# dusk-network/plonk_gadgets

Measured on AMD Instinct MI355X. Metric: gadget constraints/sec (range_check 256-bit), higher is better.
Workload: dtype u64x4 (BLS12-381 scalar, Montgomery limbs)

## Files before the change

plonk_gadgets_amd/csrc/emit.hpp:

```cpp
#pragma once

#include <type_traits>

#include "fr.hpp"

namespace pg {

constexpr int kThreads = 256;

union FrVec {
    Fr f;
    uint4 v[2];
};

struct EmitOut {
    uint4 *q[5];
    uint64_t *w[3];
    uint4 *vars;
    uint64_t gate_base, var_base;
    uint64_t zero_var;
    const uint64_t *row_off;
    const uint64_t *var_off;
    uint64_t batch;
    uint32_t tiles;
    uint32_t stride_rows;
    const uint4 *inv_dense;
    uint64_t inv_elems;
    uint32_t inv_in_place;
    uint32_t early_span, early_tiles;
};
__device__ __forceinline__ bool early_rows_candidate(const EmitOut &O, uint64_t w0, uint32_t Wt, uint32_t W, uint64_t &s0, uint64_t &s1) {
    s0 = s1 = 0;
    if (!O.early_tiles || Wt != W) return false;
    s0 = w0 - w0 % O.early_span;
    s1 = s0 + O.early_span < O.batch ? s0 + O.early_span : O.batch;
    return (w0 - s0) / W < O.early_tiles;
}

__device__ __forceinline__ void fetch_inverse(const EmitOut &O, uint64_t s, void *rec_fr) {
    uint4 *z = reinterpret_cast<uint4 *>(rec_fr);
    z[0] = O.inv_dense[s];
    z[1] = O.inv_dense[O.inv_elems + s];
}

enum : uint32_t { T_ZERO = 0, T_ONE = 1, T_NEG1 = 2, T_QC_A = 3, T_QC_B = 4, T_POW = 8 };
constexpr int kTableEntries = 8 + 256;

typedef unsigned int pg_u32x4 __attribute__((ext_vector_type(4)));

__device__ __forceinline__ void store16(uint4 *p, uint4 v) {
#if defined(PG_NT_STORES)
    pg_u32x4 t = {v.x, v.y, v.z, v.w};
    __builtin_nontemporal_store(t, reinterpret_cast<pg_u32x4 *>(p));
#else
    *p = v;
#endif
}

__device__ __forceinline__ void lds_barrier() {
#if defined(PG_FULL_BARRIERS)
    __syncthreads();
#else
    asm volatile("s_waitcnt lgkmcnt(0)\n\ts_barrier" ::: "memory");
#endif
}

__device__ __forceinline__ uint64_t uniform64(uint64_t x) {
    return (uint64_t)(uint32_t)__builtin_amdgcn_readfirstlane((int)(uint32_t)x) |
           (uint64_t)(uint32_t)__builtin_amdgcn_readfirstlane((int)(uint32_t)(x >> 32)) << 32;
}

__device__ __forceinline__ Fr lds_fr(const uint4 *table, uint32_t id) {
    FrVec t;
    t.v[0] = table[2 * id];
    t.v[1] = table[2 * id + 1];
    return t.f;
}

__device__ __forceinline__ void fill_common_table(uint4 *table, const uint4 *pow2, uint32_t tid, uint32_t entries) {
    for (uint32_t e = tid; e < entries; e += kThreads) {
        FrVec t;
        t.f = fr_zero();
        if (e == T_ONE) t.f = fr_one();
        else if (e == T_NEG1) t.f = fr_neg_one();
        else if (e >= T_POW && pow2) { t.v[0] = pow2[(e - T_POW) * 2]; t.v[1] = pow2[(e - T_POW) * 2 + 1]; }
        if (e != T_QC_A && e != T_QC_B) {
            table[2 * e] = t.v[0];
            table[2 * e + 1] = t.v[1];
        }
    }
}

template <bool SMALL_ITEMS, uint32_t UNI>
__device__ __forceinline__ uint32_t find_item(const uint32_t *off, uint32_t Wt, uint32_t r, uint32_t it, bool uniform) {
    if constexpr (UNI != 0) {
        if (uniform) return r / UNI;
    }
    if constexpr (SMALL_ITEMS) {
        uint32_t lo = it, hi = Wt;
        while (hi - lo > 1) {
            const uint32_t mid = (lo + hi) >> 1;
            if (off[mid] <= r) lo = mid; else hi = mid;
        }
        return lo;
    } else {
        while (r >= off[it + 1]) it++;
        return it;
    }
}

template <class GD, bool RAGGED = GD::kRagged>
struct UniformShape {
    static constexpr uint32_t rows = 0, vars = 0;
};
template <class GD>
struct UniformShape<GD, true> {
    static constexpr uint32_t rows = GD::kUniformRows, vars = GD::kUniformVars;
};

template <class GD, class = void>
struct Periodic {
    static constexpr bool ok = false;
};
template <class GD>
struct Periodic<GD, std::void_t<decltype(GD::kPeriodic)>> {
    static constexpr bool ok = GD::kPeriodic;
};
constexpr uint32_t periodic_wire_lanes(uint32_t R) {
    uint32_t L = 256;
    while ((2 * L) % R) L--;
    return L;
}

#ifndef PG_EMIT_WAVES_PER_SIMD
#define PG_EMIT_WAVES_PER_SIMD 1
#endif

enum EmitMode : int { EMIT_ALL = 0, EMIT_STRUCTURE = 1, EMIT_ROWS = 2, EMIT_VALUES = 3 };

template <class GD, class = void>
struct Split {
    static constexpr bool ok = false;
};
template <class GD>
struct Split<GD, std::void_t<decltype(GD::kSplit)>> {
    static constexpr bool ok = GD::kSplit;
};
template <class GD, class = void>
struct RegionVars {
    static constexpr bool ok = false;
};
template <class GD>
struct RegionVars<GD, std::void_t<decltype(GD::kRegionVars)>> {
    static constexpr bool ok = GD::kRegionVars;
};
template <class GD, class = void>
struct InvDense {
    static constexpr bool ok = false;
};
template <class GD>
struct InvDense<GD, std::void_t<decltype(GD::kInvDense)>> {
    static constexpr bool ok = GD::kInvDense;
};
template <class GD, int MODE>
struct EmitShape {
    using Rec = typename GD::ItemRec;
    static constexpr int W = GD::W;
};
template <class GD>
struct EmitShape<GD, EMIT_ROWS> {
    using Rec = typename GD::RowRec;
    static constexpr int W = GD::kRowsW;
};

constexpr uint32_t kRegionLead = 8, kRegionStage = (kRegionLead + 256 + 16) / 8 * 9;

template <class GD, int MODE = EMIT_ALL>
__global__ __launch_bounds__(kThreads, PG_EMIT_WAVES_PER_SIMD) void emit_kernel(const typename GD::Args A, const EmitOut O) {
    static_assert(MODE != EMIT_STRUCTURE || !(GD::kRagged || GD::kRecInRows), "rows of this gadget depend on its inputs");
    constexpr bool kVars = MODE == EMIT_ALL || MODE == EMIT_VALUES;
    constexpr bool kRows = MODE != EMIT_VALUES;
    constexpr int W = EmitShape<GD, MODE>::W;
    using Rec = typename EmitShape<GD, MODE>::Rec;
    constexpr uint32_t kTable = GD::kUsePow2 ? kTableEntries : T_POW;
    __shared__ uint4 s_table[kTable * 2];
    __shared__ Rec s_item[W];
    __shared__ uint32_t s_roff[W + 1], s_voff[W + 1];

    const uint32_t tid = threadIdx.x;
    {
        const uint4 *p2 = nullptr;
        if constexpr (GD::kUsePow2) p2 = GD::pow2(A);
        fill_common_table(s_table, p2, tid, kTable);
    }
    GD::fill_table(A, s_table, tid);
    lds_barrier();

    for (uint32_t t = blockIdx.x; t < O.tiles; t += gridDim.x) {
#if defined(PG_XCD_REMAP)
        const uint32_t q8 = O.tiles >> 3, r8 = O.tiles & 7, x = t & 7, k = t >> 3;
        const uint32_t tile = x * q8 + (x < r8 ? x : r8) + k;
#elif defined(PG_TILE_SPREAD)
        const uint32_t qs = O.tiles / PG_TILE_SPREAD, rs = O.tiles % PG_TILE_SPREAD, x = t % PG_TILE_SPREAD, k = t / PG_TILE_SPREAD;
        const uint32_t tile = x * qs + (x < rs ? x : rs) + k;
#else
        const uint32_t tile = t;
#endif
        const uint64_t w0 = O.stride_rows ? (uint64_t)tile : (uint64_t)tile * W;
        const uint32_t Wt = O.stride_rows ? 1u : (uint32_t)((O.batch - w0) < (uint64_t)W ? (O.batch - w0) : (uint64_t)W);
        if constexpr (MODE == EMIT_ROWS && Periodic<GD>::ok) {
            if (O.row_off[w0 + Wt] - O.row_off[w0] == (uint64_t)Wt * UniformShape<GD>::rows) continue;
        }
        uint64_t row0, var0;
        uint32_t G = 0, V = 0;
        uint64_t my_r = 0, my_v = 0, tail_r = 0, tail_v = 0;
        if constexpr (GD::kRagged) {
            row0 = O.row_off[w0];
            var0 = O.var_off[w0];
            if (tid <= Wt) {
                my_r = O.row_off[w0 + tid];
                my_v = O.var_off[w0 + tid];
            }
            if constexpr (W == kThreads) {
                if (tid == 0) {
                    tail_r = O.row_off[w0 + Wt];
                    tail_v = O.var_off[w0 + Wt];
                }
            }
        } else {
            G = GD::rows_per_item(A);
            V = GD::vars_per_item(A);
            row0 = w0 * (O.stride_rows ? O.stride_rows : G);
            var0 = w0 * V;
        }

        if constexpr ((GD::kRagged || GD::kRecInRows) && MODE != EMIT_STRUCTURE) {
            for (uint32_t i = tid; i < Wt; i += kThreads) GD::item_rows(A, O, w0 + i, s_table, s_item[i]);
        }
        if constexpr (GD::kRagged) {
            if (tid <= Wt) {
                s_roff[tid] = (uint32_t)(my_r - row0);
                s_voff[tid] = (uint32_t)(my_v - var0);
            }
            if constexpr (W == kThreads) {
                if (tid == 0) {
                    s_roff[Wt] = (uint32_t)(tail_r - row0);
                    s_voff[Wt] = (uint32_t)(tail_v - var0);
                }
            }
        }
        if constexpr (GD::kRagged || GD::kRecInRows) lds_barrier();
        if constexpr (kVars) {
            if (tid < Wt) GD::item(A, O, w0 + tid, s_table, s_item[tid]);
        }

        const uint32_t total_rows = GD::kRagged ? s_roff[Wt] : Wt * G;
        const uint32_t total_vars = GD::kRagged ? s_voff[Wt] : Wt * V;
        constexpr uint32_t kUniR = UniformShape<GD>::rows, kUniV = UniformShape<GD>::vars;
        const bool uni_rows = kUniR != 0 && total_rows == Wt * kUniR, uni_vars = kUniV != 0 && total_vars == Wt * kUniV;

        if constexpr (kRows) {
            {
                const uint32_t total = total_rows * 2;
#if defined(PG_UNALIGNED_SWEEPS)
                const uint32_t mis = 0;
#else
                const uint32_t mis = (uint32_t)((reinterpret_cast<uintptr_t>(O.q[0] + row0 * 2) >> 4) & 7u);
#endif
                const uint32_t v0 = tid < mis ? tid + kThreads : tid;
                const uint32_t h = (v0 - mis) & 1;
                uint32_t it = 0, j = (v0 - mis) >> 1;
                if constexpr (!GD::kRagged) { it = j / G; j -= it * G; }
                for (uint32_t u = v0; u < total + mis; u += kThreads) {
                    const uint32_t idx = u - mis;
                    if constexpr (GD::kRagged) {
                        const uint32_t r = idx >> 1;
                        it = find_item<W >= 64, kUniR>(s_roff, Wt, r, it, uni_rows);
                        j = uni_rows ? r - it * kUniR : r - s_roff[it];
                    }
                    uint4 v[5];
                    GD::selectors(A, s_item[it], j, s_table, h, v);
#pragma unroll
                    for (int c = 0; c < 5; c++) store16(O.q[c] + (row0 * 2 + idx), v[c]);
                    if constexpr (!GD::kRagged) {
                        j += kThreads / 2;
                        if (j >= G) { const uint32_t d = j / G; it += d; j -= d * G; }
                    }
                }
            }

#pragma unroll
            for (int c = 0; c < 3; c++) {
                uint64_t *col = O.w[c] + row0;
                const uint32_t shift = (uint32_t)((reinterpret_cast<uintptr_t>(col) >> 3) & 1);
                const uint32_t pairs = (total_rows + shift + 1) >> 1;
#if defined(PG_UNALIGNED_SWEEPS)
                const uint32_t pmis = 0;
#else
                const uint32_t pmis = (uint32_t)(((reinterpret_cast<uintptr_t>(col) - 8 * shift) >> 4) & 7u);
#endif
                uint32_t it = 0;
                for (uint32_t pv = tid < pmis ? tid + kThreads : tid; pv < pairs + pmis; pv += kThreads) {
                    const uint32_t p = pv - pmis;
                    const int64_t r0 = (int64_t)2 * p - shift;
                    uint64_t val[2];
#pragma unroll
                    for (int k = 0; k < 2; k++) {
                        const int64_t r = r0 + k;
                        uint32_t rr = r < 0 ? 0u : (uint32_t)r;
                        if (rr >= total_rows) rr = total_rows - 1;
                        uint32_t j, vo;
                        if constexpr (GD::kRagged) {
                            it = find_item<W >= 64, kUniR>(s_roff, Wt, rr, it, uni_rows);
                            j = uni_rows ? rr - it * kUniR : rr - s_roff[it];
                            vo = (uni_rows && uni_vars) ? it * kUniV : s_voff[it];
                        } else {
                            it = rr / G;
                            j = rr - it * G;
                            vo = it * V;
                        }
                        uint64_t out[3];
                        GD::wires(A, O, s_item[it], w0 + it, O.var_base + var0 + vo, j, out);
                        val[k] = out[c];
                    }
                    if (r0 >= 0 && r0 + 1 < (int64_t)total_rows) {
                        store16(reinterpret_cast<uint4 *>(col + r0),
                                make_uint4((uint32_t)val[0], (uint32_t)(val[0] >> 32), (uint32_t)val[1],
                                           (uint32_t)(val[1] >> 32)));
                    } else {
                        if (r0 >= 0) col[r0] = val[0];
                        if (r0 + 1 < (int64_t)total_rows) col[r0 + 1] = val[1];
                    }
                }
            }
        }

        lds_barrier();

        if constexpr (kVars) {
            const bool inv_here = InvDense<GD>::ok && !O.inv_in_place;
#if defined(PG_UNALIGNED_SWEEPS)
            const uint32_t smis = 0;
#else
            const uint32_t smis = (uint32_t)((reinterpret_cast<uintptr_t>(O.vars + var0 * 2) >> 5) & 3u);
#endif
#if !defined(PG_VAR_SWEEP_SINGLE)
            if constexpr (RegionVars<GD>::ok && MODE == EMIT_VALUES) {
                __shared__ uint4 s_reg[4 * kRegionStage];
                const uint32_t wave = tid >> 6, lane = tid & 63;
                uint4 *wp = s_reg + wave * kRegionStage;
                constexpr uint32_t B2 = 2 * GD::kBlocks;
                const uint32_t units = Wt * B2;
                const uint32_t tile_mis = (uint32_t)((reinterpret_cast<uintptr_t>(O.vars + var0 * 2) >> 5) & 3u);
                for (uint32_t q = wave; q < units; q += kThreads / 64) {
                    const uint32_t it = q / B2, r = q - it * B2, b = r >> 1;
                    const uint32_t kind = (r + (GD::kBlocks == 2 ? it : it >> 1)) & 1;
                    const Rec &R = s_item[it];
                    const auto &Bk = GD::region_block(R, b);
                    const uint32_t n = GD::region_n(A, R);
                    const uint32_t count = kind ? (n + 1 < 256 ? n + 1 : 256) : 256;
                    uint32_t vitem, vend;
                    if constexpr (GD::kRagged) {
                        vitem = uni_vars ? it * kUniV : s_voff[it];
                        vend = uni_vars ? vitem + kUniV : s_voff[it + 1];
                    } else {
                        vitem = it * V;
                        vend = vitem + V;
                    }
                    const uint32_t kfirst = GD::region_k(A, R, b, kind ? 257 : 1);
                    const uint32_t mis0 = (tile_mis + vitem) & 3u;
                    uint32_t ks, ke;
                    if (kind == 0) {
                        ks = b == 0 ? 0 : kfirst;
                        if (it != 0 || b != 0) ks += (4u - ((mis0 + ks) & 3u)) & 3u;
                        ke = kfirst + 256;
                        ke -= (mis0 + ke) & 3u;
                    } else {
                        ks = kfirst - ((mis0 + kfirst) & 3u);
                        ke = b + 1 < GD::kBlocks ? GD::region_k(A, R, b + 1, 1) : vend - vitem;
                        if (it + 1 != Wt || b + 1 < GD::kBlocks) ke += (4u - ((mis0 + ke) & 3u)) & 3u;
                    }
                    const uint32_t h_end = (count - 1) >> 7;
                    uint32_t hole = ~0u;
                    if (!inv_here)
                        for (uint32_t k = kfirst + count; k < ke && k < vend - vitem; k++)
                            if (GD::is_inv_slot(A, R, k)) hole = k;
                    FrVec v[4];
                    const uint32_t i0 = 4 * lane;
                    if (kind == 0) {
#pragma unroll
                        for (int t = 0; t < 4; t++) v[t].f = raw_bit(Bk.Tc, i0 + t) ? fr_one() : fr_zero();
                    } else {
                        v[0].f = fr_zero();
                        if (i0 && i0 < count) v[0].f = fr_to_mont(raw_low_bits(Bk.Tc, i0));
#pragma unroll
                        for (int t = 1; t < 4; t++) {
                            v[t].f = v[t - 1].f;
                            if (i0 + t < count && raw_bit(Bk.Tc, i0 + t - 1)) {
                                FrVec p;
                                p.v[0] = s_table[2 * (T_POW + i0 + t - 1)];
                                p.v[1] = s_table[2 * (T_POW + i0 + t - 1) + 1];
                                v[t].f = fr_add(v[t - 1].f, p.f);
                            }
                        }
                    }
                    const uint32_t npre = ks < kfirst ? kfirst - ks : 0, npost = ke > kfirst + count ? ke - (kfirst + count) : 0;
                    FrVec nb;
                    uint32_t nb_at = ~0u;
                    if (lane < npre + npost) {
                        const uint32_t k = lane < npre ? ks + lane : kfirst + count + (lane - npre);
                        const uint32_t vitem_n = vend - vitem;
                        nb.f = k < vitem_n ? GD::var_value(A, R, s_table, k) : GD::var_value(A, s_item[it + 1], s_table, k - vitem_n);
                        nb_at = kRegionLead + 2 * (k - kfirst) - (lane < npre ? 0 : 256 * h_end);
                    }
#pragma unroll
                    for (int h = 0; h < 2; h++) {
                        if ((lane >> 5) == (uint32_t)h) {
                            const uint32_t u0 = kRegionLead + 8 * (lane & 31), w0 = u0 + (u0 >> 3);
#pragma unroll
                            for (int t = 0; t < 4; t++) {
                                wp[w0 + 2 * t] = v[t].v[0];
                                wp[w0 + 2 * t + 1] = v[t].v[1];
                            }
                        }
                        if (h == 1 && lane == 31) {
#pragma unroll
                            for (int t = 0; t < 4; t++) {
                                wp[kRegionLead - 8 + 2 * t] = v[t].v[0];
                                wp[kRegionLead - 8 + 2 * t + 1] = v[t].v[1];
                            }
                        }
                        if (nb_at != ~0u && (lane < npre ? h == 0 : (uint32_t)h == h_end)) {
                            wp[nb_at + (nb_at >> 3)] = nb.v[0];
                            wp[nb_at + 1 + ((nb_at + 1) >> 3)] = nb.v[1];
                        }
                        asm volatile("" ::: "memory");
                        const uint32_t mid = kfirst + 128 - ((mis0 + kfirst + 128) & 3u);
                        const uint32_t lo = h == 0 ? ks : mid, hi = (uint32_t)h == h_end ? ke : (h == 0 ? mid : lo);
                        const uint32_t total = hi > lo ? 2 * (hi - lo) : 0;
                        uint4 *dst = O.vars + ((uint64_t)var0 + vitem + lo) * 2;
                        const uint32_t mis = (uint32_t)((reinterpret_cast<uintptr_t>(dst) >> 4) & 7u);
                        const uint32_t lead = kRegionLead + 2 * (lo - kfirst) - 256 * h;
#pragma unroll
                        for (int j = 0; j < 5; j++) {
                            const uint32_t g = 64 * j + lane - mis;
                            const uint32_t u = g + lead;
                            if (g < total && lo + (g >> 1) != hole) store16(dst + g, wp[u + (u >> 3)]);
                        }
                        asm volatile("" ::: "memory");
                    }
                }
            } else
#endif
            {
            const uint32_t sv0 = tid < smis ? tid + kThreads : tid;
                uint32_t it = 0, k = sv0 - smis;
                if constexpr (!GD::kRagged) { it = k / V; k -= it * V; }
                for (uint32_t sv = sv0; sv < total_vars + smis; sv += kThreads) {
                    const uint32_t s = sv - smis;
                    if constexpr (GD::kRagged) {
                        it = find_item<W >= 64, kUniV>(s_voff, Wt, s, it, uni_vars);
                        k = uni_vars ? s - it * kUniV : s - s_voff[it];
                    }
                    uint4 *dst = O.vars + (var0 + s) * 2;
                    if (inv_here || !GD::is_inv_slot(A, s_item[it], k)) {
                        FrVec val;
                        val.f = GD::var_value(A, s_item[it], s_table, k);
                        store16(dst, val.v[0]);
                        store16(dst + 1, val.v[1]);
                    }
                    if constexpr (!GD::kRagged) {
                        k += kThreads;
                        if (k >= V) { const uint32_t d = k / V; it += d; k -= d * V; }
                    }
                }
            }
            }
        lds_barrier();
    }
}

#ifndef PG_ROWS_WAVES_PER_SIMD
#define PG_ROWS_WAVES_PER_SIMD 8
#endif
template <class GD>
__device__ __forceinline__ void periodic_tile_rows(const typename GD::Args &A, const EmitOut &O, const uint4 v[5], uint32_t tid, uint64_t w0,
                                                   uint32_t Wt, uint64_t row0, uint64_t var0) {
    constexpr uint32_t R = GD::kUniformRows, VV = GD::kUniformVars;
    constexpr uint32_t IPP = (kThreads / 2) / R, LS = IPP * R * 2;
    constexpr uint32_t LW = periodic_wire_lanes(R), IPW = 2 * LW / R;
    typename GD::RowRec full{};
    const uint32_t total_rows = Wt * R;
    if (tid < LS) {
        const uint32_t passes = (total_rows * 2 + LS - 1) / LS;
        uint4 *base[5];
        uint32_t at[5];
#pragma unroll
        for (int c = 0; c < 5; c++) {
            base[c] = O.q[c] + (row0 * 2 + tid);
            at[c] = (uint32_t)(((uint64_t)c * passes) / 5);
        }
        for (uint32_t p = 0; p < passes; p++) {
#pragma unroll
            for (int c = 0; c < 5; c++) {
                const uint32_t off = at[c] * LS;
                if (off + tid < total_rows * 2) store16(base[c] + off, v[c]);
                at[c] = at[c] + 1 == passes ? 0 : at[c] + 1;
            }
        }
    }
#pragma unroll
    for (int c = 0; c < 3; c++) {
        uint64_t *col = O.w[c] + row0;
        const uint32_t shift = (uint32_t)((reinterpret_cast<uintptr_t>(col) >> 3) & 1);
        if (tid < LW) {
            uint64_t wbase[2], slope[2];
#pragma unroll
            for (int k = 0; k < 2; k++) {
                const int32_t r = (int32_t)(2 * tid + k) - (int32_t)shift;
                const int32_t it = r < 0 ? -1 : r / (int32_t)R;
                const uint32_t j = (uint32_t)(r - it * (int32_t)R);
                const uint64_t vb = O.var_base + var0 + (uint64_t)(int64_t)it * VV;
                uint64_t a[3], b[3];
                GD::wires(A, O, full, w0 + (uint64_t)(int64_t)it, vb, j, a);
                GD::wires(A, O, full, w0 + (uint64_t)(int64_t)it, vb + 1, j, b);
                wbase[k] = a[c];
                slope[k] = b[c] - a[c];
            }
            const uint64_t step = (uint64_t)IPW * VV;
            uint64_t adv = 0;
            for (int64_t r0 = (int64_t)2 * tid - shift; r0 < (int64_t)total_rows; r0 += 2 * LW, adv += step) {
                const uint64_t v0 = wbase[0] + slope[0] * adv, v1 = wbase[1] + slope[1] * adv;
                if (r0 >= 0 && r0 + 1 < (int64_t)total_rows) {
                    store16(reinterpret_cast<uint4 *>(col + r0),
                            make_uint4((uint32_t)v0, (uint32_t)(v0 >> 32), (uint32_t)v1, (uint32_t)(v1 >> 32)));
                } else {
                    if (r0 >= 0) col[r0] = v0;
                    if (r0 + 1 < (int64_t)total_rows) col[r0 + 1] = v1;
                }
            }
        }
    }
}
template <class GD>
__device__ __forceinline__ void periodic_lane_selectors(const typename GD::Args &A, const uint4 *table, uint32_t tid, uint4 v[5]) {
    constexpr uint32_t R = GD::kUniformRows, IPP = (kThreads / 2) / R, LS = IPP * R * 2;
    typename GD::RowRec full{};
    const uint32_t rl = (tid < LS ? tid : 0) >> 1;
    GD::selectors(A, full, rl - (rl / R) * R, table, tid & 1, v);
}

template <class GD>
__global__ __launch_bounds__(kThreads, PG_ROWS_WAVES_PER_SIMD) void rows_periodic_kernel(const typename GD::Args A, const EmitOut O) {
    constexpr int W = GD::kRowsW;
    constexpr uint32_t R = GD::kUniformRows;
    __shared__ uint4 s_table[T_POW * 2];
    const uint32_t tid = threadIdx.x;
#if defined(PG_ROWS_SETPRIO)
    __builtin_amdgcn_s_setprio(PG_ROWS_SETPRIO);
#endif
    fill_common_table(s_table, nullptr, tid, T_POW);
    GD::fill_table(A, s_table, tid);
    lds_barrier();
    uint4 v[5];
    periodic_lane_selectors<GD>(A, s_table, tid, v);

    for (uint32_t tile = blockIdx.x; tile < O.tiles; tile += gridDim.x) {
        const uint64_t w0 = (uint64_t)tile * W;
        const uint32_t Wt = (uint32_t)((O.batch - w0) < (uint64_t)W ? (O.batch - w0) : (uint64_t)W);
        uint64_t s0, s1;
        const bool cand = early_rows_candidate(O, w0, Wt, W, s0, s1);
        const uint64_t span_rows = cand ? O.row_off[s1] - O.row_off[s0] : 0;
        const uint64_t row0 = uniform64(O.row_off[w0]), var0 = uniform64(O.var_off[w0]), row1 = uniform64(O.row_off[w0 + Wt]);
        if (row1 - row0 != Wt * R) continue;
        if (cand && uniform64(span_rows) == (s1 - s0) * R) continue;
        periodic_tile_rows<GD>(A, O, v, tid, w0, Wt, row0, var0);
    }
}

__global__ __launch_bounds__(kThreads) void fill_kernel(uint4 *dst, uint64_t n16, uint32_t streams, uint64_t pattern) {
    const uint4 v = make_uint4((uint32_t)pattern, (uint32_t)(pattern >> 32), (uint32_t)~pattern, (uint32_t)(~pattern >> 32));
    const uint64_t part = n16 / streams;
    constexpr uint64_t kPiece = 65536;
    for (uint64_t base = (uint64_t)blockIdx.x * kPiece; base < part; base += (uint64_t)gridDim.x * kPiece) {
        const uint64_t end = base + kPiece < part ? base + kPiece : part;
        for (uint64_t i = base + threadIdx.x; i < end; i += kThreads)
            for (uint32_t s = 0; s < streams; s++) store16(dst + (uint64_t)s * part + i, v);
    }
    if (blockIdx.x == 0)
        for (uint64_t i = part * streams + threadIdx.x; i < n16; i += kThreads) store16(dst + i, v);
}

constexpr uint32_t kFillOneshotLds = 160 * 1024 / 2 - 1024;
constexpr uint32_t kFillOneshotUnits = 2 * kThreads;
__global__ __launch_bounds__(kThreads) void fill_oneshot_kernel(uint4 *dst, uint64_t n16, uint64_t pattern) {
    extern __shared__ uint4 fill_oneshot_pad[];
    const uint4 v = make_uint4((uint32_t)pattern, (uint32_t)(pattern >> 32), (uint32_t)~pattern, (uint32_t)(~pattern >> 32));
    const uint64_t base = (uint64_t)blockIdx.x * kFillOneshotUnits + threadIdx.x;
#pragma unroll
    for (uint32_t k = 0; k < kFillOneshotUnits / kThreads; k++)
        if (base + k * kThreads < n16) store16(dst + base + k * kThreads, v);
    if (n16 == ~0ull) fill_oneshot_pad[threadIdx.x] = v;
}

__global__ __launch_bounds__(kThreads) void fill_columns_kernel(EmitOut O, uint64_t n_gates, uint64_t n_vars, uint64_t rows_per_tile,
                                                                uint64_t vars_per_tile, uint64_t pattern) {
    const uint4 v = make_uint4((uint32_t)pattern, (uint32_t)(pattern >> 32), (uint32_t)~pattern, (uint32_t)(~pattern >> 32));
    for (uint64_t tile = blockIdx.x; tile < O.tiles; tile += gridDim.x) {
        const uint64_t r0 = tile * rows_per_tile, r1 = r0 + rows_per_tile < n_gates ? r0 + rows_per_tile : n_gates;
        const uint64_t v0 = tile * vars_per_tile, v1 = tile + 1 == O.tiles ? n_vars : (v0 + vars_per_tile < n_vars ? v0 + vars_per_tile : n_vars);
        if (r0 < r1) {
            for (uint64_t u = 2 * r0 + threadIdx.x; u < 2 * r1; u += kThreads) {
#pragma unroll
                for (int c = 0; c < 5; c++) store16(O.q[c] + u, v);
            }
            for (uint64_t u = r0 / 2 + threadIdx.x; u < r1 / 2; u += kThreads) {
#pragma unroll
                for (int c = 0; c < 3; c++) store16(reinterpret_cast<uint4 *>(O.w[c]) + u, v);
            }
            if ((r1 & 1) && threadIdx.x == 0)
                for (int c = 0; c < 3; c++) O.w[c][r1 - 1] = pattern;
        }
        for (uint64_t u = 2 * v0 + threadIdx.x; u < 2 * v1; u += kThreads) store16(O.vars + u, v);
    }
}

__global__ __launch_bounds__(kThreads) void from_canonical_kernel(const uint4 *raw, uint64_t n, uint4 *out, uint8_t *bad_mask,
                                                                 uint32_t *bad_count) {
    const uint64_t i = (uint64_t)blockIdx.x * kThreads + threadIdx.x;
    if (i >= n) return;
    FrVec x;
    x.v[0] = raw[2 * i];
    x.v[1] = raw[2 * i + 1];
    const Fr q = fr_modulus();
    bool ge = true;
    for (int k = 3; k >= 0; k--)
        if (x.f.l[k] != q.l[k]) { ge = x.f.l[k] > q.l[k]; break; }
    FrVec r;
    r.f = ge ? fr_zero() : fr_to_mont(x.f);
    out[2 * i] = r.v[0];
    out[2 * i + 1] = r.v[1];
    if (bad_mask) bad_mask[i] = ge ? 1 : 0;
    if (ge) atomicAdd(bad_count, 1u);
}
__global__ __launch_bounds__(kThreads) void to_canonical_kernel(const uint4 *in, uint64_t n, uint4 *raw) {
    const uint64_t i = (uint64_t)blockIdx.x * kThreads + threadIdx.x;
    if (i >= n) return;
    FrVec x, r;
    x.v[0] = in[2 * i];
    x.v[1] = in[2 * i + 1];
    r.f = fr_from_mont(x.f);
    raw[2 * i] = r.v[0];
    raw[2 * i + 1] = r.v[1];
}

constexpr int kScanBlock = 1024;

__device__ __forceinline__ uint64_t block_exclusive_scan(uint64_t v, uint64_t *s_warp, uint64_t &block_total) {
    const uint32_t lane = threadIdx.x & 63, wave = threadIdx.x >> 6;
    uint64_t incl = v;
#pragma unroll
    for (int d = 1; d < 64; d <<= 1) {
        uint64_t t = __shfl_up(incl, d, 64);
        if (lane >= (uint32_t)d) incl += t;
    }
    if (lane == 63) s_warp[wave] = incl;
    __syncthreads();
    uint64_t base = 0;
    for (uint32_t wv = 0; wv < wave; wv++) base += s_warp[wv];
    block_total = s_warp[0] + s_warp[1] + s_warp[2] + s_warp[3];
    __syncthreads();
    return base + incl - v;
}

__global__ __launch_bounds__(kThreads) void scan_top_kernel(uint64_t *blk_rows, uint64_t *blk_vars, uint32_t nblk) {
    __shared__ uint64_t s_warp[4];
    uint64_t carry_r = 0, carry_v = 0;
    for (uint32_t base = 0; base < nblk; base += kThreads) {
        uint32_t i = base + threadIdx.x;
        uint64_t r = i < nblk ? blk_rows[i] : 0, v = i < nblk ? blk_vars[i] : 0, tr, tv;
        uint64_t er = block_exclusive_scan(r, s_warp, tr);
        uint64_t ev = block_exclusive_scan(v, s_warp, tv);
        if (i < nblk) { blk_rows[i] = carry_r + er; blk_vars[i] = carry_v + ev; }
        carry_r += tr;
        carry_v += tv;
    }
}

struct PlanTotals {
    uint64_t n_gates, n_vars;
    uint32_t errs, pad;
};


struct PlanScan {
    unsigned long long *agg;
    uint64_t *blk_rows, *blk_vars;
    uint64_t *row_off, *var_off;
    PlanTotals *host;
    uint32_t *err_count;
    uint32_t blocks_cap;
    uint32_t fused;
};
constexpr unsigned long long kAggA = 1ull << 63, kAggP = 1ull << 62;
constexpr uint32_t kPlanFusedBlocks = 2048;
constexpr uint32_t kPlanSpinLimit = 1u << 22;

__device__ __forceinline__ unsigned long long plan_rmw_read(unsigned long long *p) {
    return __hip_atomic_fetch_add(p, 0ull, __ATOMIC_RELAXED, __HIP_MEMORY_SCOPE_AGENT);
}
__device__ __forceinline__ void plan_publish(unsigned long long *p, unsigned long long flag, uint64_t rows, uint64_t vars) {
    __hip_atomic_exchange(p, flag | rows << 31 | vars, __ATOMIC_RELAXED, __HIP_MEMORY_SCOPE_AGENT);
}
__device__ __forceinline__ uint64_t wave_sum(uint64_t x) {
#pragma unroll
// ... 146 lines not shown
```

plonk_gadgets_amd/csrc/range_gadgets.hpp:

```cpp
#pragma once

#include "emit.hpp"
#include "footprint.hpp"
#include "invert.hpp"

namespace pg {

struct alignas(16) BoundRec {
    Fr Tm;
    Fr Tc;
    Fr UZ[2];
};

__device__ __forceinline__ void bound_fetch_z(const EmitOut &O, uint64_t s, BoundRec &b) { fetch_inverse(O, s, &b.UZ[1]); }

__device__ __forceinline__ Fr bound_u(const Fr &Tm, const Fr &Tc, uint32_t n) {
    if (!raw_has_high_bits(Tc, n)) return fr_zero();
    return fr_sub(fr_to_mont(raw_low_bits(Tc, n)), Tm);
}

__device__ __forceinline__ uint32_t bound_item(const Fr &Tm, uint32_t n, BoundRec &b) {
    const Fr Tc = fr_from_mont(Tm);
    b.Tm = Tm;
    b.Tc = Tc;
    const Fr u = bound_u(Tm, Tc, n);
    b.UZ[0] = u;
    return fr_is_zero(u) ? 1u : 0u;
}

__device__ __forceinline__ uint32_t bound_z_offset(uint32_t n) { return 259 + n; }

__device__ __forceinline__ void bound_selector_ids(uint32_t jj, uint32_t n, bool is_min, uint32_t id[5]) {
    uint32_t qm = T_ZERO, ql = T_ZERO, qr = T_ZERO, qo = T_NEG1, qc = T_ZERO;
    if (jj >= 2 && jj < 2 * n + 2) {
        if (jj & 1) {
            ql = T_POW + ((jj - 3) >> 1);
            qr = T_ONE;
        } else {
            qm = T_ONE;
        }
    } else if (jj == 0) {
        ql = is_min ? T_ONE : T_NEG1;
        qc = is_min ? T_QC_B : T_QC_A;
    } else if (jj == 1) {
        ql = T_ONE;
        qo = T_ZERO;
    } else if (jj == 2 * n + 2) {
        ql = T_ONE;
        qr = T_NEG1;
    } else if (jj == 2 * n + 3) {
        qm = T_NEG1;
        qc = T_ONE;
    } else {
        qm = T_ONE;
        qo = T_ZERO;
    }
    id[0] = qm; id[1] = ql; id[2] = qr; id[3] = qo; id[4] = qc;
}

constexpr uint32_t kWitnessWire = 0xffffffffu;

__device__ __forceinline__ void bound_wire_offsets(uint32_t jj, uint32_t n, uint32_t vb, uint32_t x, uint32_t off[3]) {
    uint32_t a, b, c;
    if (jj >= 2 && jj < 2 * n + 2) {
        const uint32_t i = (jj - 2) >> 1;
        a = vb + 1 + i;
        if (jj & 1) { b = vb + 257 + i; c = vb + 258 + i; }
        else { b = a; c = a; }
    } else if (jj == 0) {
        a = x; b = x; c = vb;
    } else if (jj == 1) {
        a = b = c = vb + 257;
    } else if (jj == 2 * n + 2) {
        a = vb + 257 + n; b = vb; c = vb + 258 + n;
    } else if (jj == 2 * n + 3) {
        a = vb + 259 + n; b = vb + 258 + n; c = vb + 260 + n;
    } else {
        a = vb + 260 + n; b = vb + 258 + n; c = b;
    }
    off[0] = a; off[1] = b; off[2] = c;
}

__device__ __forceinline__ Fr bound_var_value(const BoundRec &B, uint32_t y, uint32_t kk, uint32_t n) {
    if (kk == 0) return B.Tm;
    if (kk <= 256) return raw_bit(B.Tc, kk - 1) ? fr_one() : fr_zero();
    if (kk <= 257 + n) {
        const uint32_t i = kk - 257;
        return i ? fr_to_mont(raw_low_bits(B.Tc, i)) : fr_zero();
    }
    if (kk <= 259 + n) {
        const uint4 *p = reinterpret_cast<const uint4 *>(B.UZ) + 2 * (kk - (258 + n));
        FrVec v;
        v.v[0] = p[0];
        v.v[1] = p[1];
        return v.f;
    }
    return y ? fr_one() : fr_zero();
}

__device__ __forceinline__ void ids_to_values(const uint32_t id[5], const uint4 *table, uint32_t h, uint4 out[5]) {
#pragma unroll
    for (int c = 0; c < 5; c++) out[c] = table[2 * id[c] + h];
}

struct RangeCheckGD {
    struct Args {
        Fr min_range, max_range;
        uint32_t n;
        const uint4 *witness;
        const uint64_t *witness_vars;
        uint64_t *result_vars;
        const uint4 *pow2;
    };
    static constexpr int kInv = 2;
    static constexpr bool kInvDense = true;
    static constexpr int kInvGroup = 4;
    __device__ static void inv_operands(const Args &A, const EmitOut &, uint64_t item, uint32_t, FrVec &p, FrVec &q, uint32_t &) {
        p.v[0] = A.witness[item * 2];
        p.v[1] = A.witness[item * 2 + 1];
        q.f = p.f;
    }
    __device__ static Fr inv_combine(const Args &A, uint32_t e, const Fr &x, const Fr &, uint32_t) {
        const Fr t0 = fr_sub(fr_sub(A.max_range, fr_one()), x), t1 = fr_sub(x, A.min_range);
        Fr Tm;
#pragma unroll
        for (int i = 0; i < 4; i++) Tm.l[i] = e == 0 ? t0.l[i] : t1.l[i];
        return bound_u(Tm, fr_from_mont(Tm), A.n);
    }
    __device__ static uint4 *inv_slot(const Args &A, const EmitOut &O, uint64_t item, uint32_t e) {
        const uint64_t V = 2 * A.n + 523 + (A.witness_vars ? 0u : 1u), VB = A.n + 261;
        return O.vars + 2 * (item * V + (A.witness_vars ? 0u : 1u) + e * VB + bound_z_offset(A.n));
    }
    struct alignas(16) ItemRec {
        Fr x;
        BoundRec b[2];
        uint32_t y[2];
        uint32_t pad[2];
    };
    __device__ static bool is_inv_slot(const Args &A, const ItemRec &, uint32_t k) {
        const uint32_t x0 = A.witness_vars ? 0u : 1u, VB = A.n + 261, z = bound_z_offset(A.n);
        return k == x0 + z || k == x0 + VB + z;
    }
#ifndef PG_RC_W
#define PG_RC_W 32
#endif
    static constexpr int W = PG_RC_W;
    static constexpr bool kRagged = false, kRecInRows = false, kUsePow2 = true;

    __device__ static const uint4 *pow2(const Args &A) { return A.pow2; }
    __device__ static uint32_t rows_per_item(const Args &A) { return 4 * A.n + 11; }
    __device__ static uint32_t xo(const Args &A) { return A.witness_vars ? 0u : 1u; }
    __device__ static uint32_t vars_per_item(const Args &A) { return 2 * A.n + 523 + xo(A); }

    __device__ static void fill_table(const Args &A, uint4 *table, uint32_t tid) {
        if (tid == T_QC_A || tid == T_QC_B) {
            FrVec t;
            t.f = tid == T_QC_A ? fr_sub(A.max_range, fr_one())
                                : fr_neg(A.min_range);
            table[2 * tid] = t.v[0];
            table[2 * tid + 1] = t.v[1];
        }
    }

    __device__ static void item(const Args &A, const EmitOut &O, uint64_t item, const uint4 *table, ItemRec &R) {
        FrVec x;
        x.v[0] = A.witness[item * 2];
        x.v[1] = A.witness[item * 2 + 1];
        R.x = x.f;
        bound_fetch_z(O, item, R.b[0]);
        bound_fetch_z(O, O.batch + item, R.b[1]);
        R.y[0] = bound_item(fr_sub(lds_fr(table, T_QC_A), x.f), A.n, R.b[0]);
        R.y[1] = bound_item(fr_add(x.f, lds_fr(table, T_QC_B)), A.n, R.b[1]);
        const uint64_t V = vars_per_item(A);
        if (A.result_vars) A.result_vars[item] = O.var_base + item * V + (V - 1);
    }

    __device__ static void selectors(const Args &A, const ItemRec &, uint32_t j, const uint4 *table, uint32_t h, uint4 out[5]) {
        const uint32_t L = 2 * A.n + 5;
        uint32_t id[5];
        if (j == 2 * L) {
            id[0] = T_ONE; id[1] = T_ZERO; id[2] = T_ZERO; id[3] = T_NEG1; id[4] = T_ZERO;
        } else {
            const bool is_min = j >= L;
            bound_selector_ids(is_min ? j - L : j, A.n, is_min, id);
        }
        ids_to_values(id, table, h, out);
    }

    __device__ static void wires(const Args &A, const EmitOut &, const ItemRec &, uint64_t item, uint64_t vbase, uint32_t j,
                                 uint64_t out[3]) {
        const uint32_t n = A.n, L = 2 * n + 5, VB = n + 261, x0 = xo(A);
        uint32_t off[3];
        if (j == 2 * L) {
            off[0] = x0 + 260 + n;
            off[1] = x0 + VB + 260 + n;
            off[2] = x0 + 2 * VB;
        } else {
            const bool is_min = j >= L;
            bound_wire_offsets(is_min ? j - L : j, n, is_min ? x0 + VB : x0, kWitnessWire, off);
        }
        const uint64_t xvar = A.witness_vars ? A.witness_vars[item] : vbase;
#pragma unroll
        for (int c = 0; c < 3; c++) out[c] = off[c] == kWitnessWire ? xvar : vbase + off[c];
    }

    __device__ static Fr var_value(const Args &A, const ItemRec &R, const uint4 *, uint32_t k) {
        const uint32_t n = A.n, VB = n + 261;
        if (!A.witness_vars) {
            if (k == 0) return R.x;
            k -= 1;
        }
        if (k == 2 * VB) return (R.y[0] & R.y[1]) ? fr_one() : fr_zero();
        uint32_t kk = k, blk = 0;
        if (kk >= VB) { kk -= VB; blk = 1; }
        return bound_var_value(R.b[blk], R.y[blk], kk, n);
    }
    static constexpr bool kRegionVars = true;
    static constexpr uint32_t kBlocks = 2;
    __device__ static uint32_t region_n(const Args &A, const ItemRec &) { return A.n; }
    __device__ static const BoundRec &region_block(const ItemRec &R, uint32_t b) { return R.b[b]; }
    __device__ static uint32_t region_k(const Args &A, const ItemRec &, uint32_t b, uint32_t kk) { return xo(A) + b * (A.n + 261) + kk; }
};

struct RangeBoundsGD {
    struct Args {
        const uint4 *min_range_v, *max_range_v;
        const uint32_t *num_bits_v;
        const uint4 *witness;
        uint64_t *result_vars;
        const uint4 *pow2;
    };
    static constexpr int kInv = 2;
    static constexpr bool kInvDense = true;
    static constexpr int kInvGroup = 4;
    __device__ static void inv_operands(const Args &A, const EmitOut &, uint64_t item, uint32_t e, FrVec &p, FrVec &q, uint32_t &n) {
        const uint4 *bound = e == 0 ? A.max_range_v : A.min_range_v;
        p.v[0] = A.witness[item * 2];
        p.v[1] = A.witness[item * 2 + 1];
        q.v[0] = bound[item * 2];
        q.v[1] = bound[item * 2 + 1];
        n = A.num_bits_v[item];
    }
    __device__ static Fr inv_combine(const Args &, uint32_t e, const Fr &x, const Fr &m, uint32_t n) {
        const Fr t0 = fr_sub(fr_sub(m, fr_one()), x), t1 = fr_sub(x, m);
        Fr Tm;
#pragma unroll
        for (int i = 0; i < 4; i++) Tm.l[i] = e == 0 ? t0.l[i] : t1.l[i];
        return bound_u(Tm, fr_from_mont(Tm), n);
    }
    __device__ static uint4 *inv_slot(const Args &A, const EmitOut &O, uint64_t item, uint32_t e) {
        const uint32_t n = A.num_bits_v[item];
        return O.vars + 2 * (O.var_off[item] + 1 + e * (n + 261) + bound_z_offset(n));
    }
    struct alignas(16) ItemRec {
        Fr x;
        Fr qc[2];
        BoundRec b[2];
        uint32_t y[2];
        uint32_t n, pad;
    };
    static constexpr int W = PG_RC_W;
    static constexpr bool kRagged = true, kRecInRows = true, kUsePow2 = true;
    static constexpr uint32_t kUniformRows = 0, kUniformVars = 0;

    __device__ static const uint4 *pow2(const Args &A) { return A.pow2; }
    __device__ static void fill_table(const Args &, uint4 *table, uint32_t tid) {
        if (tid == T_QC_A || tid == T_QC_B) {
            table[2 * tid] = make_uint4(0, 0, 0, 0);
            table[2 * tid + 1] = make_uint4(0, 0, 0, 0);
        }
    }
    __device__ static void item_rows(const Args &A, const EmitOut &, uint64_t item, const uint4 *, ItemRec &R) {
        FrVec mx, mn;
        mx.v[0] = A.max_range_v[item * 2];
        mx.v[1] = A.max_range_v[item * 2 + 1];
        mn.v[0] = A.min_range_v[item * 2];
        mn.v[1] = A.min_range_v[item * 2 + 1];
        R.qc[0] = fr_sub(mx.f, fr_one());
        R.qc[1] = fr_neg(mn.f);
        R.n = A.num_bits_v[item];
    }
    __device__ static void item(const Args &A, const EmitOut &O, uint64_t item, const uint4 *, ItemRec &R) {
        FrVec x;
        x.v[0] = A.witness[item * 2];
        x.v[1] = A.witness[item * 2 + 1];
        R.x = x.f;
        const uint32_t n = R.n;
        bound_fetch_z(O, item, R.b[0]);
        bound_fetch_z(O, O.batch + item, R.b[1]);
        R.y[0] = bound_item(fr_sub(R.qc[0], x.f), n, R.b[0]);
        R.y[1] = bound_item(fr_add(x.f, R.qc[1]), n, R.b[1]);
        if (A.result_vars) A.result_vars[item] = O.var_base + O.var_off[item] + (2 * n + 523);
    }
    __device__ static void selectors(const Args &, const ItemRec &R, uint32_t j, const uint4 *table, uint32_t h, uint4 out[5]) {
        const uint32_t L = 2 * R.n + 5;
        uint32_t id[5];
        if (j == 2 * L) {
            id[0] = T_ONE; id[1] = T_ZERO; id[2] = T_ZERO; id[3] = T_NEG1; id[4] = T_ZERO;
        } else {
            const bool is_min = j >= L;
            bound_selector_ids(is_min ? j - L : j, R.n, is_min, id);
        }
        ids_to_values(id, table, h, out);
        if (id[4] == T_QC_A || id[4] == T_QC_B) out[4] = reinterpret_cast<const uint4 *>(R.qc)[2 * (id[4] - T_QC_A) + h];
    }
    __device__ static void wires(const Args &, const EmitOut &, const ItemRec &R, uint64_t, uint64_t vbase, uint32_t j, uint64_t out[3]) {
        const uint32_t n = R.n, L = 2 * n + 5, VB = n + 261;
        uint32_t off[3];
        if (j == 2 * L) {
            off[0] = 1 + 260 + n;
            off[1] = 1 + VB + 260 + n;
            off[2] = 1 + 2 * VB;
        } else {
            const bool is_min = j >= L;
            bound_wire_offsets(is_min ? j - L : j, n, is_min ? 1 + VB : 1, kWitnessWire, off);
        }
#pragma unroll
        for (int c = 0; c < 3; c++) out[c] = off[c] == kWitnessWire ? vbase : vbase + off[c];
    }
    __device__ static bool is_inv_slot(const Args &, const ItemRec &R, uint32_t k) {
        const uint32_t VB = R.n + 261, z = bound_z_offset(R.n);
        return k == 1 + z || k == 1 + VB + z;
    }
    __device__ static Fr var_value(const Args &, const ItemRec &R, const uint4 *, uint32_t k) {
        const uint32_t n = R.n, VB = n + 261;
        if (k == 0) return R.x;
        k -= 1;
        if (k == 2 * VB) return (R.y[0] & R.y[1]) ? fr_one() : fr_zero();
        uint32_t kk = k, blk = 0;
        if (kk >= VB) { kk -= VB; blk = 1; }
        return bound_var_value(R.b[blk], R.y[blk], kk, n);
    }
    static constexpr bool kRegionVars = true;
    static constexpr uint32_t kBlocks = 2;
    __device__ static uint32_t region_n(const Args &, const ItemRec &R) { return R.n; }
    __device__ static const BoundRec &region_block(const ItemRec &R, uint32_t b) { return R.b[b]; }
    __device__ static uint32_t region_k(const Args &, const ItemRec &R, uint32_t b, uint32_t kk) { return 1 + b * (R.n + 261) + kk; }
};

template <bool RAGGED>
struct MaxBoundGD {
    struct Args {
        Fr max_range;
        uint32_t n;
        const uint4 *max_range_v;
        const uint32_t *num_bits_v;
        const uint4 *witness;
        const uint64_t *witness_vars;
        uint64_t *result_vars;
        const uint4 *pow2;
    };
    static constexpr int kInv = 1;
    static constexpr bool kInvDense = true;
    static constexpr int kInvGroup = 4;
    __device__ static uint4 *inv_slot(const Args &A, const EmitOut &O, uint64_t item, uint32_t) {
        const uint32_t n = RAGGED ? A.num_bits_v[item] : A.n;
        const uint32_t x0 = (!RAGGED && A.witness_vars) ? 0u : 1u;
        const uint64_t first = RAGGED ? O.var_off[item] : item * (uint64_t)(n + 261 + x0);
        return O.vars + 2 * (first + x0 + bound_z_offset(n));
    }
    __device__ static void inv_operands(const Args &A, const EmitOut &, uint64_t item, uint32_t, FrVec &p, FrVec &q, uint32_t &n) {
        p.v[0] = A.witness[item * 2];
        p.v[1] = A.witness[item * 2 + 1];
        n = A.n;
        q.f = A.max_range;
        if constexpr (RAGGED) {
            q.v[0] = A.max_range_v[item * 2];
            q.v[1] = A.max_range_v[item * 2 + 1];
            n = A.num_bits_v[item];
        }
    }
    __device__ static Fr inv_combine(const Args &, uint32_t, const Fr &x, const Fr &m, uint32_t n) {
        const Fr Tm = fr_sub(fr_sub(m, fr_one()), x);
        return bound_u(Tm, fr_from_mont(Tm), n);
    }
    struct alignas(16) ItemRec {
        Fr x;
        Fr qc;
        BoundRec b;
        uint32_t y, n;
        uint32_t pad[2];
    };
#ifndef PG_MB_W
#define PG_MB_W 16
#endif
    static constexpr int W = PG_MB_W;
    static constexpr bool kRagged = RAGGED, kRecInRows = RAGGED, kUsePow2 = true;

    __device__ static const uint4 *pow2(const Args &A) { return A.pow2; }
    __device__ static uint32_t rows_per_item(const Args &A) { return 2 * A.n + 5; }
    __device__ static uint32_t xo(const Args &A) { return (!RAGGED && A.witness_vars) ? 0u : 1u; }
    __device__ static uint32_t vars_per_item(const Args &A) { return A.n + 261 + xo(A); }

    __device__ static void fill_table(const Args &A, uint4 *table, uint32_t tid) {
        if (tid == T_QC_A) {
            FrVec t;
            t.f = RAGGED ? fr_zero() : fr_sub(A.max_range, fr_one());
            table[2 * tid] = t.v[0];
            table[2 * tid + 1] = t.v[1];
        } else if (tid == T_QC_B) {
            table[2 * tid] = make_uint4(0, 0, 0, 0);
            table[2 * tid + 1] = make_uint4(0, 0, 0, 0);
        }
    }

    static constexpr uint32_t kUniformRows = 0, kUniformVars = 0;
    __device__ static void item_rows(const Args &A, const EmitOut &, uint64_t item, const uint4 *, ItemRec &R) {
        FrVec m;
        m.v[0] = A.max_range_v[item * 2];
        m.v[1] = A.max_range_v[item * 2 + 1];
        R.qc = fr_sub(m.f, fr_one());
        R.n = A.num_bits_v[item];
    }

    __device__ static void item(const Args &A, const EmitOut &O, uint64_t item, const uint4 *table, ItemRec &R) {
        FrVec x;
        x.v[0] = A.witness[item * 2];
        x.v[1] = A.witness[item * 2 + 1];
        R.x = x.f;
        bound_fetch_z(O, item, R.b);
        uint32_t n = A.n;
        Fr qc;
        if constexpr (RAGGED) {
            qc = R.qc;
            n = R.n;
        } else {
            qc = lds_fr(table, T_QC_A);
            R.qc = qc;
            R.n = n;
        }
        R.y = bound_item(fr_sub(qc, x.f), n, R.b);
        if (A.result_vars) {
            const uint64_t first = RAGGED ? O.var_off[item] : item * (uint64_t)(n + 261 + xo(A));
            A.result_vars[item] = O.var_base + first + (n + 260 + xo(A));
        }
    }

    __device__ static void selectors(const Args &A, const ItemRec &R, uint32_t j, const uint4 *table, uint32_t h, uint4 out[5]) {
        uint32_t id[5];
        bound_selector_ids(j, RAGGED ? R.n : A.n, false, id);
        ids_to_values(id, table, h, out);
        if constexpr (RAGGED) {
            if (j == 0) {
                FrVec q;
                q.f = R.qc;
                out[4] = q.v[h];
            }
        }
    }

    __device__ static void wires(const Args &A, const EmitOut &, const ItemRec &R, uint64_t item, uint64_t vbase, uint32_t j,
                                 uint64_t out[3]) {
        uint32_t off[3];
        bound_wire_offsets(j, RAGGED ? R.n : A.n, xo(A), kWitnessWire, off);
        const uint64_t xvar = xo(A) ? vbase : A.witness_vars[item];
#pragma unroll
        for (int c = 0; c < 3; c++) out[c] = off[c] == kWitnessWire ? xvar : vbase + off[c];
    }

    __device__ static bool is_inv_slot(const Args &A, const ItemRec &R, uint32_t k) {
        return k == xo(A) + bound_z_offset(RAGGED ? R.n : A.n);
    }
    __device__ static Fr var_value(const Args &A, const ItemRec &R, const uint4 *, uint32_t k) {
        if (xo(A)) {
            if (k == 0) return R.x;
            k -= 1;
        }
        return bound_var_value(R.b, R.y, k, RAGGED ? R.n : A.n);
    }
    static constexpr bool kRegionVars = true;
    static constexpr uint32_t kBlocks = 1;
    __device__ static uint32_t region_n(const Args &A, const ItemRec &R) { return RAGGED ? R.n : A.n; }
    __device__ static const BoundRec &region_block(const ItemRec &R, uint32_t) { return R.b; }
    __device__ static uint32_t region_k(const Args &A, const ItemRec &, uint32_t, uint32_t kk) { return xo(A) + kk; }
};

struct DecompositionGD {
    struct Args {
        uint32_t n;
        const uint4 *witness;
        const uint64_t *witness_vars;
        uint64_t *result_vars;
        const uint4 *pow2;
    };
    static constexpr int kInv = 1;
    static constexpr bool kInvDense = true;
    static constexpr int kInvGroup = 4;
    __device__ static void inv_operands(const Args &A, const EmitOut &, uint64_t item, uint32_t, FrVec &p, FrVec &q, uint32_t &) {
        p.v[0] = A.witness[item * 2];
        p.v[1] = A.witness[item * 2 + 1];
        q.f = p.f;
    }
    __device__ static Fr inv_combine(const Args &A, uint32_t, const Fr &x, const Fr &, uint32_t) {
        return bound_u(x, fr_from_mont(x), A.n);
    }
    __device__ static uint4 *inv_slot(const Args &A, const EmitOut &O, uint64_t item, uint32_t) {
        return O.vars + 2 * (item * (uint64_t)(A.n + 260) + bound_z_offset(A.n) - 1);
    }
    struct alignas(16) ItemRec {
        BoundRec b;
        uint32_t y, pad[3];
    };
    static constexpr int W = 32;
    static constexpr bool kRagged = false, kRecInRows = false, kUsePow2 = true;
    __device__ static const uint4 *pow2(const Args &A) { return A.pow2; }
    __device__ static uint32_t rows_per_item(const Args &A) { return 2 * A.n + 4; }
    __device__ static uint32_t vars_per_item(const Args &A) { return A.n + 260; }
    __device__ static void fill_table(const Args &, uint4 *table, uint32_t tid) {
        if (tid == T_QC_A || tid == T_QC_B) {
            table[2 * tid] = make_uint4(0, 0, 0, 0);
            table[2 * tid + 1] = make_uint4(0, 0, 0, 0);
        }
    }
    __device__ static void item(const Args &A, const EmitOut &O, uint64_t item, const uint4 *, ItemRec &R) {
        FrVec x;
        x.v[0] = A.witness[item * 2];
        x.v[1] = A.witness[item * 2 + 1];
        bound_fetch_z(O, item, R.b);
        R.y = bound_item(x.f, A.n, R.b);
        const uint64_t V = vars_per_item(A);
        if (A.result_vars) A.result_vars[item] = O.var_base + item * V + (V - 1);
    }
    __device__ static void selectors(const Args &A, const ItemRec &, uint32_t j, const uint4 *table, uint32_t h, uint4 out[5]) {
        uint32_t id[5];
        bound_selector_ids(j + 1, A.n, false, id);
        ids_to_values(id, table, h, out);
    }
    __device__ static void wires(const Args &A, const EmitOut &, const ItemRec &, uint64_t item, uint64_t vbase, uint32_t j,
                                 uint64_t out[3]) {
        uint32_t off[3];
        bound_wire_offsets(j + 1, A.n, kWitnessWire, kWitnessWire, off);
        const uint64_t xvar = A.witness_vars[item];
#pragma unroll
        for (int c = 0; c < 3; c++) out[c] = off[c] == kWitnessWire ? xvar : vbase + off[c];
    }
    __device__ static bool is_inv_slot(const Args &A, const ItemRec &, uint32_t k) { return k + 1 == bound_z_offset(A.n); }
    __device__ static Fr var_value(const Args &A, const ItemRec &R, const uint4 *, uint32_t k) {
        return bound_var_value(R.b, R.y, k + 1, A.n);
    }
    static constexpr bool kRegionVars = true;
    static constexpr uint32_t kBlocks = 1;
    __device__ static uint32_t region_n(const Args &A, const ItemRec &) { return A.n; }
    __device__ static const BoundRec &region_block(const ItemRec &R, uint32_t) { return R.b; }
    __device__ static uint32_t region_k(const Args &, const ItemRec &, uint32_t, uint32_t kk) { return kk - 1; }
};

template <uint32_t KIND>
__global__ __launch_bounds__(kThreads) void max_bound_plan_kernel(const uint4 *max_range, uint64_t batch, const uint4 *pow2,
                                                                 uint32_t *num_bits, uint32_t *rows, uint32_t *vars, const PlanScan P) {
    constexpr uint32_t kR0 = kind_rows(KIND), kR1 = kind_rows(KIND, 1) - kR0, kV0 = kind_vars(KIND), kV1 = kind_vars(KIND, 1) - kV0;
    uint32_t r[4] = {0, 0, 0, 0}, v[4] = {0, 0, 0, 0};
#pragma unroll
    for (int k = 0; k < 4; k++) {
        const uint64_t i = (uint64_t)blockIdx.x * kScanBlock + threadIdx.x * 4 + k;
        if (i < batch) {
            FrVec m, p;
            m.v[0] = max_range[i * 2];
            m.v[1] = max_range[i * 2 + 1];
            const Fr mm1 = fr_sub(m.f, fr_one());
            uint32_t nb = raw_bit_length(fr_from_mont(mm1));
            if (nb < 1) nb = 1;
            p.v[0] = pow2[nb * 2];
            p.v[1] = pow2[nb * 2 + 1];
            uint32_t n = raw_bit_length(fr_from_mont(p.f));
            if (n < 1) n = 1;
            num_bits[i] = n;
            r[k] = kR0 + kR1 * n;
            v[k] = kV0 + kV1 * n;
        }
    }
    plan_store(P, r, v, batch, rows, vars);
}

__global__ void pow2_table_kernel(uint4 *out) {
    if (threadIdx.x != 0 || blockIdx.x != 0) return;
    FrVec p;
    p.f = fr_one();
    for (int i = 0; i < 256; i++) {
        out[2 * i] = p.v[0];
        out[2 * i + 1] = p.v[1];
        p.f = fr_add(p.f, p.f);
    }
}

}
```

Before: 32.65 billion.

## Specialise region-sweep emit: occupancy bound, uniform wave index, cheap neighbour values

The region-vars EMIT_VALUES instantiation now gets its own launch-bounds occupancy target of four waves per SIMD. The wave index is forced into a scalar register with readfirstlane. Neighbour variable lookups in the region sweep use a specialised path that returns Tm instead of computing a Montgomery conversion of the low bits for accumulator slots. The occupancy hint and the scalar wave index aim to cut register pressure and divergence. The neighbour shortcut assumes those boundary slots only ever need Tm, which may be wrong if a neighbour falls inside the accumulator range.

```diff
diff --git a/plonk_gadgets_amd/csrc/emit.hpp b/plonk_gadgets_amd/csrc/emit.hpp
--- a/plonk_gadgets_amd/csrc/emit.hpp
+++ b/plonk_gadgets_amd/csrc/emit.hpp
@@ -175,8 +175,13 @@
 
 constexpr uint32_t kRegionLead = 8, kRegionStage = (kRegionLead + 256 + 16) / 8 * 9;
 
+constexpr int kRegionWavesPerSimd = 4;
+template <class GD, int MODE>
+constexpr int emit_waves_per_simd() {
+    return RegionVars<GD>::ok && MODE == EMIT_VALUES ? kRegionWavesPerSimd : PG_EMIT_WAVES_PER_SIMD;
+}
 template <class GD, int MODE = EMIT_ALL>
-__global__ __launch_bounds__(kThreads, PG_EMIT_WAVES_PER_SIMD) void emit_kernel(const typename GD::Args A, const EmitOut O) {
+__global__ __launch_bounds__(kThreads, (emit_waves_per_simd<GD, MODE>())) void emit_kernel(const typename GD::Args A, const EmitOut O) {
     static_assert(MODE != EMIT_STRUCTURE || !(GD::kRagged || GD::kRecInRows), "rows of this gadget depend on its inputs");
     constexpr bool kVars = MODE == EMIT_ALL || MODE == EMIT_VALUES;
     constexpr bool kRows = MODE != EMIT_VALUES;
@@ -347,7 +352,9 @@
 #if !defined(PG_VAR_SWEEP_SINGLE)
             if constexpr (RegionVars<GD>::ok && MODE == EMIT_VALUES) {
                 __shared__ uint4 s_reg[4 * kRegionStage];
-                const uint32_t wave = tid >> 6, lane = tid & 63;
+                uint32_t rtid = tid;
+                asm volatile("" : "+v"(rtid));
+                const uint32_t wave = __builtin_amdgcn_readfirstlane(rtid >> 6), lane = rtid & 63;
                 uint4 *wp = s_reg + wave * kRegionStage;
                 constexpr uint32_t B2 = 2 * GD::kBlocks;
                 const uint32_t units = Wt * B2;
@@ -410,7 +417,8 @@
                     if (lane < npre + npost) {
                         const uint32_t k = lane < npre ? ks + lane : kfirst + count + (lane - npre);
                         const uint32_t vitem_n = vend - vitem;
-                        nb.f = k < vitem_n ? GD::var_value(A, R, s_table, k) : GD::var_value(A, s_item[it + 1], s_table, k - vitem_n);
+                        const bool own = k < vitem_n;
+                        nb.f = GD::region_neighbour(A, own ? R : s_item[it + 1], own ? k : k - vitem_n);
                         nb_at = kRegionLead + 2 * (k - kfirst) - (lane < npre ? 0 : 256 * h_end);
                     }
 #pragma unroll
diff --git a/plonk_gadgets_amd/csrc/range_gadgets.hpp b/plonk_gadgets_amd/csrc/range_gadgets.hpp
--- a/plonk_gadgets_amd/csrc/range_gadgets.hpp
+++ b/plonk_gadgets_amd/csrc/range_gadgets.hpp
@@ -81,10 +81,12 @@
     off[0] = a; off[1] = b; off[2] = c;
 }
 
+template <bool NEIGHBOUR = false>
 __device__ __forceinline__ Fr bound_var_value(const BoundRec &B, uint32_t y, uint32_t kk, uint32_t n) {
     if (kk == 0) return B.Tm;
     if (kk <= 256) return raw_bit(B.Tc, kk - 1) ? fr_one() : fr_zero();
     if (kk <= 257 + n) {
+        if constexpr (NEIGHBOUR) return B.Tm;
         const uint32_t i = kk - 257;
         return i ? fr_to_mont(raw_low_bits(B.Tc, i)) : fr_zero();
     }
@@ -204,7 +206,8 @@
         for (int c = 0; c < 3; c++) out[c] = off[c] == kWitnessWire ? xvar : vbase + off[c];
     }
 
-    __device__ static Fr var_value(const Args &A, const ItemRec &R, const uint4 *, uint32_t k) {
+    template <bool NEIGHBOUR>
+    __device__ static Fr value_of(const Args &A, const ItemRec &R, uint32_t k) {
         const uint32_t n = A.n, VB = n + 261;
         if (!A.witness_vars) {
             if (k == 0) return R.x;
@@ -213,10 +216,12 @@
         if (k == 2 * VB) return (R.y[0] & R.y[1]) ? fr_one() : fr_zero();
         uint32_t kk = k, blk = 0;
         if (kk >= VB) { kk -= VB; blk = 1; }
-        return bound_var_value(R.b[blk], R.y[blk], kk, n);
-    }
+        return bound_var_value<NEIGHBOUR>(R.b[blk], R.y[blk], kk, n);
+    }
+    __device__ static Fr var_value(const Args &A, const ItemRec &R, const uint4 *, uint32_t k) { return value_of<false>(A, R, k); }
     static constexpr bool kRegionVars = true;
     static constexpr uint32_t kBlocks = 2;
+    __device__ static Fr region_neighbour(const Args &A, const ItemRec &R, uint32_t k) { return value_of<true>(A, R, k); }
     __device__ static uint32_t region_n(const Args &A, const ItemRec &) { return A.n; }
     __device__ static const BoundRec &region_block(const ItemRec &R, uint32_t b) { return R.b[b]; }
     __device__ static uint32_t region_k(const Args &A, const ItemRec &, uint32_t b, uint32_t kk) { return xo(A) + b * (A.n + 261) + kk; }
@@ -322,17 +327,20 @@
         const uint32_t VB = R.n + 261, z = bound_z_offset(R.n);
         return k == 1 + z || k == 1 + VB + z;
     }
-    __device__ static Fr var_value(const Args &, const ItemRec &R, const uint4 *, uint32_t k) {
+    template <bool NEIGHBOUR>
+    __device__ static Fr value_of(const ItemRec &R, uint32_t k) {
         const uint32_t n = R.n, VB = n + 261;
         if (k == 0) return R.x;
         k -= 1;
         if (k == 2 * VB) return (R.y[0] & R.y[1]) ? fr_one() : fr_zero();
         uint32_t kk = k, blk = 0;
         if (kk >= VB) { kk -= VB; blk = 1; }
-        return bound_var_value(R.b[blk], R.y[blk], kk, n);
-    }
+        return bound_var_value<NEIGHBOUR>(R.b[blk], R.y[blk], kk, n);
+    }
+    __device__ static Fr var_value(const Args &, const ItemRec &R, const uint4 *, uint32_t k) { return value_of<false>(R, k); }
     static constexpr bool kRegionVars = true;
     static constexpr uint32_t kBlocks = 2;
+    __device__ static Fr region_neighbour(const Args &, const ItemRec &R, uint32_t k) { return value_of<true>(R, k); }
     __device__ static uint32_t region_n(const Args &, const ItemRec &R) { return R.n; }
     __device__ static const BoundRec &region_block(const ItemRec &R, uint32_t b) { return R.b[b]; }
     __device__ static uint32_t region_k(const Args &, const ItemRec &R, uint32_t b, uint32_t kk) { return 1 + b * (R.n + 261) + kk; }
@@ -461,15 +469,18 @@
     __device__ static bool is_inv_slot(const Args &A, const ItemRec &R, uint32_t k) {
         return k == xo(A) + bound_z_offset(RAGGED ? R.n : A.n);
     }
-    __device__ static Fr var_value(const Args &A, const ItemRec &R, const uint4 *, uint32_t k) {
+    template <bool NEIGHBOUR>
+    __device__ static Fr value_of(const Args &A, const ItemRec &R, uint32_t k) {
         if (xo(A)) {
             if (k == 0) return R.x;
             k -= 1;
         }
-        return bound_var_value(R.b, R.y, k, RAGGED ? R.n : A.n);
-    }
+        return bound_var_value<NEIGHBOUR>(R.b, R.y, k, RAGGED ? R.n : A.n);
+    }
+    __device__ static Fr var_value(const Args &A, const ItemRec &R, const uint4 *, uint32_t k) { return value_of<false>(A, R, k); }
     static constexpr bool kRegionVars = true;
     static constexpr uint32_t kBlocks = 1;
+    __device__ static Fr region_neighbour(const Args &A, const ItemRec &R, uint32_t k) { return value_of<true>(A, R, k); }
     __device__ static uint32_t region_n(const Args &A, const ItemRec &R) { return RAGGED ? R.n : A.n; }
     __device__ static const BoundRec &region_block(const ItemRec &R, uint32_t) { return R.b; }
     __device__ static uint32_t region_k(const Args &A, const ItemRec &, uint32_t, uint32_t kk) { return xo(A) + kk; }
@@ -540,6 +551,7 @@
     }
     static constexpr bool kRegionVars = true;
     static constexpr uint32_t kBlocks = 1;
+    __device__ static Fr region_neighbour(const Args &A, const ItemRec &R, uint32_t k) { return bound_var_value<true>(R.b, R.y, k + 1, A.n); }
     __device__ static uint32_t region_n(const Args &A, const ItemRec &) { return A.n; }
     __device__ static const BoundRec &region_block(const ItemRec &R, uint32_t) { return R.b; }
     __device__ static uint32_t region_k(const Args &, const ItemRec &, uint32_t, uint32_t kk) { return kk - 1; }
```

New measurement: 32.55 billion. No clear change (-0.3%).
